# gauravchak/two_tower_models

Hardware: AMD Instinct MI355X
Metric: user-item pairs/sec (in-batch softmax train step: fwd + zero_grad + bwd + dense-exact Adam) (higher is better)
Workload: dtype f32

## Files before the change

### include/tt_hotpath.h

```cpp
#ifndef TT_HOTPATH_H
#define TT_HOTPATH_H

#include <stdint.h>

#ifdef __cplusplus
extern "C" {
#endif

#define TT_ABI_VERSION 6

#define TT_E_BADARG (-1)
#define TT_E_WORKSPACE (-2)
#define TT_E_UNSUPPORTED (-3)

typedef void* tt_stream_t;

int tt_abi_version(void);
const char* tt_last_error_string(void);

int tt_profile_enable(int on);
int tt_profile_read(const char* kernel, double* total_ms, int64_t* launches);
int tt_profile_filter(const char* kernels);
int tt_profile_pause(int paused);

int tt_gather_rows(const float* table, int64_t n_rows, int64_t dim, const int64_t* ids,
                   int64_t n_ids, float* out, int64_t ld_out, int32_t* oob_flag,
                   tt_stream_t stream);

#define TT_GEMM_NT 0
#define TT_GEMM_NN 1
#define TT_GEMM_TN 2
#define TT_EPI_NONE 0
#define TT_EPI_RELU 1
#define TT_EPI_RELU_MASK 2
int64_t tt_gemm_workspace_bytes(int layout, int64_t M, int64_t N, int64_t K);
int tt_gemm_f32(int layout, int64_t M, int64_t N, int64_t K, const float* A, int64_t lda,
                const float* B, int64_t ldb, float* C, int64_t ldc, const float* bias,
                int epilogue, const float* aux, int64_t ldaux, int accumulate, void* ws,
                int64_t ws_bytes, tt_stream_t stream);
int tt_gemm_tn_colsum_f32(int64_t M, int64_t N, int64_t K, const float* A, int64_t lda, const float* B,
                          int64_t ldb, float* C, int64_t ldc, int accumulate, float* a_colsum, void* ws,
                          int64_t ws_bytes, tt_stream_t stream);

int64_t tt_colsum_workspace_bytes(int64_t M, int64_t N);
int tt_colsum_f32(const float* X, int64_t M, int64_t N, int64_t ldx, float* out, void* ws,
                  int64_t ws_bytes, tt_stream_t stream);

typedef struct {
  const float* table; int64_t n_rows; const int64_t* ids; const float* feats; int64_t ldf; int64_t F;
  const float *W1, *b1, *W2, *b2, *W3, *b3;
  float* y; int64_t ldy; float* h_out; float* tin_out;
  const float* extra; int64_t ldx;
} tt_tower_fwd_side;
typedef struct {
  const float* dy; int64_t ldy; const float *W2, *W3, *h;
  float* d_emb; int64_t ld_demb; float* d_f; float* dh;
  float* d_extra; int64_t ld_dx;
} tt_tower_bwd_side;
typedef struct {
  const float* dy; int64_t ldy; const float *tin, *d_f, *h, *dh, *feats; int64_t ldf; int64_t F;
  float *dW1, *db1, *dW2, *db2, *dW3, *db3;
  void* ws; int64_t ws_bytes;
  const float* extra; int64_t ldx;
} tt_tower_wgrad_side;
int tt_tower_supported(int64_t D, int64_t F, int64_t hidden, int64_t d_out, int64_t E);
// ... 323 lines not shown
```

### two_tower_models_amd/_native.py

```python
from __future__ import annotations

import ctypes as C
import os
from typing import Optional

import torch

_PKG = os.path.dirname(os.path.abspath(__file__))
LIB_PATH = os.path.join(_PKG, "lib", "libtt_hotpath.so")

TT_GEMM_NT, TT_GEMM_NN, TT_GEMM_TN = 0, 1, 2
TT_EPI_NONE, TT_EPI_RELU, TT_EPI_RELU_MASK = 0, 1, 2
TT_F32, TT_BF16, TT_F16X2 = 0, 1, 2
TT_E_BADARG, TT_E_WORKSPACE, TT_E_UNSUPPORTED = -1, -2, -3
TT_DEBIAS_COMBINED, TT_DEBIAS_POSITION, TT_DEBIAS_USER = 0, 1, 2
TT_COMM_ID_BYTES = 128
TT_COMM_F32, TT_COMM_I32, TT_COMM_I64, TT_COMM_U8 = 0, 1, 2, 3
TT_COMM_SUM, TT_COMM_MAX = 0, 1
TT_MAX_GRAD_SOURCES = 4
ABI_VERSION = 6

_vp, _i64, _i32, _int = C.c_void_p, C.c_int64, C.c_int32, C.c_int


# ... 32 lines not shown
                ("extra", _vp), ("ldx", _i64)]


class TowerBwdSide(C.Structure):

    _fields_ = [("dy", _vp), ("ldy", _i64), ("W2", _vp), ("W3", _vp), ("h", _vp), ("d_emb", _vp), ("ld_demb", _i64), ("d_f", _vp),
                ("dh", _vp), ("d_extra", _vp), ("ld_dx", _i64)]


class TowerWgradSide(C.Structure):

    _fields_ = [("dy", _vp), ("ldy", _i64), ("tin", _vp), ("d_f", _vp), ("h", _vp), ("dh", _vp), ("feats", _vp), ("ldf", _i64),
                ("F", _i64), ("dW1", _vp), ("db1", _vp), ("dW2", _vp), ("db2", _vp), ("dW3", _vp), ("db3", _vp), ("ws", _vp),
                ("ws_bytes", _i64), ("extra", _vp), ("ldx", _i64)]


class PlanJob(C.Structure):

    _fields_ = [("ids", _vp), ("n_ids", _i64), ("n_rows", _i64), ("sorted_ids", _vp), ("perm", _vp), ("seg_begin", _vp), ("n_unique", _vp)]


TT_PLAN_MAX_JOBS = 4
TT_ROUTE_MAX_JOBS = 8


class RouteJob(C.Structure):

    _fields_ = [("ids", _vp), ("n_ids", _i64), ("n_rows", _i64), ("rows_per_rank", _i64), ("counts", _vp), ("max_count", _vp),
                ("ws", _vp), ("ws_bytes", _i64), ("cap", _i64), ("send_ids", _vp), ("slot_of", _vp), ("src_of", _vp)]


class RouteServeJob(C.Structure):

    _fields_ = [("ids", _vp), ("n_ids", _i64), ("lo", _i64), ("n_local", _i64), ("local", _vp), ("table", _vp), ("dtype", _int),
                ("dim", _i64), ("rows", _vp)]


SIGNATURES = {
    "tt_abi_version": (_int, []),
    "tt_last_error_string": (C.c_char_p, []),
    "tt_profile_enable": (_int, [_int]),
    "tt_profile_read": (_int, [C.c_char_p, C.POINTER(C.c_double), C.POINTER(_i64)]),
    "tt_profile_filter": (_int, [C.c_char_p]),
    "tt_profile_pause": (_int, [_int]),
    "tt_gather_rows": (_int, [_vp, _i64, _i64, _vp, _i64, _vp, _i64, _vp, _vp]),
    "tt_gemm_workspace_bytes": (_i64, [_int, _i64, _i64, _i64]),
    "tt_gemm_f32": (_int, [_int, _i64, _i64, _i64, _vp, _i64, _vp, _i64, _vp, _i64, _vp, _int, _vp,
                           _i64, _int, _vp, _i64, _vp]),
    "tt_gemm_tn_colsum_f32": (_int, [_i64, _i64, _i64, _vp, _i64, _vp, _i64, _vp, _i64, _int, _vp, _vp, _i64, _vp]),
    "tt_colsum_workspace_bytes": (_i64, [_i64, _i64]),
    "tt_colsum_f32": (_int, [_vp, _i64, _i64, _i64, _vp, _vp, _i64, _vp]),
    "tt_tower_supported": (_int, [_i64, _i64, _i64, _i64, _i64]),
    "tt_tower_fwd": (_int, [C.POINTER(TowerFwdSide), _i32, _i64, _i64, _i64, _i64, _vp, _vp]),
    "tt_tower_bwd_data": (_int, [C.POINTER(TowerBwdSide), _i32, _i64, _i64, _i64, _i64, _vp]),
    "tt_tower_bwd_weights_workspace_bytes": (_i64, [_i64, _i64, _i64, _i64, _i64]),
    "tt_tower_bwd_weights": (_int, [C.POINTER(TowerWgradSide), _i32, _i64, _i64, _i64, _i64, _vp]),
    "tt_adam_begin_ids": (_int, [_vp, _vp, _i64, C.POINTER(AdamStashJob), _i32, _vp]),
    "tt_adam_begin_ids_planes": (_int, [_vp, _vp, _i64, C.POINTER(AdamStashJob), _i32, _i32, _vp]),
    "tt_adam_tables_finish": (_int, [C.POINTER(AdamFinishJob), _i32, _vp, _vp]),
    "tt_inbatch_ce_fwd_du_loss": (_int, [_vp, _i64, _vp, _i64, _i64, _i64, _i64, _i64, _vp, _i64, _vp, _vp, _vp, _vp, _i64, _vp, _vp,
                                         _vp, _vp, _i64, _vp]),
    "tt_scale_rows_g": (_int, [_vp, _i64, _vp, _vp, _i64, _i64, _vp, _i64, _vp, _vp]),
    "tt_inbatch_ce_workspace_bytes": (_i64, [_i64, _i64, _i64]),
    "tt_inbatch_ce_fwd": (_int, [_vp, _i64, _vp, _i64, _i64, _i64, _i64, _i64, _vp, _vp, _vp, _i64, _vp]),
    "tt_inbatch_ce_bwd": (_int, [_vp, _i64, _vp, _i64, _i64, _i64, _i64, _i64, _vp, _vp, _vp, _i64, _vp,
                                 _i64, _vp, _i64, _vp]),
    "tt_inbatch_ce_fwd_du": (_int, [_vp, _i64, _vp, _i64, _i64, _i64, _i64, _i64, _vp, _vp, _vp, _i64, _vp, _i64, _vp]),
    "tt_inbatch_ce_logits_bytes": (_i64, [_i64, _i64]),
    "tt_inbatch_ce_fwd_du_keep": (_int, [_vp, _i64, _vp, _i64, _i64, _i64, _i64, _i64, _vp, _vp, _vp, _i64, _vp, _i64,
                                         _vp, _i64, _vp]),
    "tt_inbatch_ce_bwd_kept": (_int, [_vp, _i64, _i64, _i64, _i64, _i64, _vp, _vp, _vp, _i64, _vp, _i64, _vp, _i64, _vp]),
    "tt_inbatch_ce_bias_workspace_bytes": (_i64, [_i64, _i64, _i64]),
# ... 255 lines not shown
```

### two_tower_models_amd/csrc/attention_wg.hip

```cpp
#include <stdlib.h>

#include "common.hpp"

namespace tt {

typedef float f32x16 __attribute__((ext_vector_type(16)));

namespace awg {
constexpr int ROWS = 56, LD = 36, IMG = ROWS * LD;
constexpr int SLD = 68, SCR = ROWS * SLD;
constexpr int HEADS = 4, DH = 32, D = 128;
__device__ __forceinline__ int arow(int e, int h) { return (e & 3) + 8 * (e >> 2) + 4 * h; }
}

struct AttnWgArgs {
  const float* qkv;
  const float* ctx;
  const float* lse;
  const float* d_ctx;
  float* d_qkv;
  int64_t B;
  int H;
};

// ... 112 lines not shown
  float4 vf[2][4];
  auto fetch_v = [&](int64_t bb) {
    const char* __restrict__ vb = reinterpret_cast<const char*>(p.qkv + bb * H * (3 * D));
#pragma unroll
    for (int t = 0; t < 2; ++t) {
      const int j = 32 * t + r;
      const bool ok = j < H;
      const unsigned vo = (unsigned)((ok ? j : 0) * (3 * D) + 2 * D + DH * head + 4 * h2) * 4u;
#pragma unroll
      for (int g = 0; g < 4; ++g) {
        const float4 x = *reinterpret_cast<const float4*>(vb + vo + 32u * g);
        vf[t][g] = ok ? x : make_float4(0.f, 0.f, 0.f, 0.f);
      }
    }
  };
  int64_t b = blockIdx.x;
  if (b < p.B) fetch_v(b);
  __syncthreads();
  for (; b < p.B; b += gridDim.x) {
    __syncthreads();
    __syncthreads();
    const int64_t bn = b + gridDim.x;
    float* __restrict__ ob = p.d_qkv + (b * H) * (3 * D);
#pragma unroll
    for (int t = 0; t < 2; ++t) {
      const int jrow = 32 * t + r;
      const bool jvalid = jrow < H;
      const int jr = jrow < ROWS ? jrow : ROWS - 1;
      const float* const ka = Kh + jr * LD + 4 * h2;
      f32x16 dv, dk;
#pragma unroll
      for (int e = 0; e < 16; ++e) { dv[e] = 0.f; dk[e] = 0.f; }
#pragma unroll
      for (int it = 0; it < 2; ++it) {
        const int ir = (32 * it + r) < ROWS ? 32 * it + r : ROWS - 1;
        f32x16 s, dp;
#pragma unroll
        for (int e = 0; e < 16; ++e) { s[e] = 0.f; dp[e] = 0.f; }
        const float* qa = Qh + ir * LD + 4 * h2;
        const float* ga = Gh + ir * LD + 4 * h2;
#pragma unroll
        for (int g = 0; g < 4; ++g) {
          const float4 a = *reinterpret_cast<const float4*>(qa + 8 * g);
          const float4 kq = *reinterpret_cast<const float4*>(ka + 8 * g);
          const float4 c = *reinterpret_cast<const float4*>(ga + 8 * g);
          s = __builtin_amdgcn_mfma_f32_32x32x2f32(a.x, kq.x, s, 0, 0, 0);
// ... 3 lines not shown
          dp = __builtin_amdgcn_mfma_f32_32x32x2f32(c.x, vf[t][g].x, dp, 0, 0, 0);
          dp = __builtin_amdgcn_mfma_f32_32x32x2f32(c.y, vf[t][g].y, dp, 0, 0, 0);
          dp = __builtin_amdgcn_mfma_f32_32x32x2f32(c.z, vf[t][g].z, dp, 0, 0, 0);
          dp = __builtin_amdgcn_mfma_f32_32x32x2f32(c.w, vf[t][g].w, dp, 0, 0, 0);
        }
#pragma unroll
        for (int q = 0; q < 4; ++q) {
          const float4 l4 = *reinterpret_cast<const float4*>(Lh + 32 * it + 8 * q + 4 * h2);
          const float4 d4 = *reinterpret_cast<const float4*>(Dh + 32 * it + 8 * q + 4 * h2);
          const float lv[4] = {l4.x, l4.y, l4.z, l4.w}, dl[4] = {d4.x, d4.y, d4.z, d4.w};
#pragma unroll
          for (int c = 0; c < 4; ++c) {
            const int e = 4 * q + c;
            const float pe = jvalid ? __expf(s[e] - lv[c]) : 0.f;
            s[e] = pe;
            dp[e] = pe * (dp[e] - dl[c]);
          }
        }
        const float* gy = Gh + (32 * it + 4 * h2) * LD + r;
        const float* qy = Qh + (32 * it + 4 * h2) * LD + r;
#pragma unroll
        for (int e = 0; e < 16; ++e) {
          const int ro = (e & 3) + 8 * (e >> 2);
          if (it == 1 && ro + 4 >= ROWS - 32) {
            const int i = 32 + ro + 4 * h2;
            const int ic = i < ROWS ? i : ROWS - 1;
            dv = __builtin_amdgcn_mfma_f32_32x32x2f32(s[e], Gh[ic * LD + r], dv, 0, 0, 0);
            dk = __builtin_amdgcn_mfma_f32_32x32x2f32(dp[e], Qh[ic * LD + r], dk, 0, 0, 0);
          } else {
            dv = __builtin_amdgcn_mfma_f32_32x32x2f32(s[e], gy[ro * LD], dv, 0, 0, 0);
            dk = __builtin_amdgcn_mfma_f32_32x32x2f32(dp[e], qy[ro * LD], dk, 0, 0, 0);
          }
        }
        if (jrow < ROWS) {
#pragma unroll
          for (int q = 0; q < 4; ++q)
            *reinterpret_cast<float4*>(Sh + jrow * SLD + 32 * it + 8 * q + 4 * h2) =
                make_float4(dp[4 * q], dp[4 * q + 1], dp[4 * q + 2], dp[4 * q + 3]);
        }
      }
      const unsigned oc = (unsigned)((32 * t + 4 * h2) * (3 * D) + DH * head + r);
#pragma unroll
      for (int e = 0; e < 16; ++e) {
        const int ro = (e & 3) + 8 * (e >> 2);
        if (32 * t + 4 * h2 + ro < H) {
          ob[oc + (unsigned)(ro * 3 * D + 2 * D)] = dv[e];
          ob[oc + (unsigned)(ro * 3 * D + D)] = dk[e];
        }
      }
    }
    if (bn < p.B) fetch_v(bn);
    __builtin_amdgcn_wave_barrier();

#pragma unroll
    for (int it = 0; it < 2; ++it) {
      f32x16 dq;
#pragma unroll
      for (int e = 0; e < 16; ++e) dq[e] = 0.f;
      const float* sy = Sh + (4 * h2) * SLD + 32 * it + r;
      const float* ky = Kh + (4 * h2) * LD + r;
#pragma unroll
      for (int jt = 0; jt < 2; ++jt) {
#pragma unroll
        for (int e = 0; e < 16; ++e) {
          if (jt == 1 && (e >> 2) == 3) continue;
          const int ro = 32 * jt + (e & 3) + 8 * (e >> 2);
          dq = __builtin_amdgcn_mfma_f32_32x32x2f32(sy[ro * SLD], ky[ro * LD], dq, 0, 0, 0);
        }
      }
      const unsigned oc = (unsigned)((32 * it + 4 * h2) * (3 * D) + DH * head + r);
#pragma unroll
      for (int e = 0; e < 16; ++e) {
        const int ro = (e & 3) + 8 * (e >> 2);
        if (32 * it + 4 * h2 + ro < H) ob[oc + (unsigned)(ro * 3 * D)] = dq[e] * scale;
      }
    }
    __syncthreads();
  }
}

bool attn_bwd_wg_supported(const void* qkv, const void* ctx, const void* d_ctx, const void* d_qkv, int64_t H, int64_t D,
                           int64_t heads) {
  const uintptr_t al = reinterpret_cast<uintptr_t>(qkv) | reinterpret_cast<uintptr_t>(ctx) | reinterpret_cast<uintptr_t>(d_ctx) |
                       reinterpret_cast<uintptr_t>(d_qkv);
  return (al & 15) == 0 && heads == awg::HEADS && D == awg::D && H >= 1 && H <= 50;
}

int attn_bwd_wg(const float* qkv, const float* ctx, const float* lse, const float* d_ctx, int64_t B, int64_t H, float* d_qkv,
                hipStream_t st) {
  AttnWgArgs a{qkv, ctx, lse, d_ctx, d_qkv, B, (int)H};
  const unsigned grid = (unsigned)(B < 256 ? B : 256);
  ProfScope prof("attn_bwd_wg_kernel", st);
  attn_bwd_wg_kernel<<<grid, 512, 0, st>>>(a);
// ... 5 lines not shown
```

### two_tower_models_amd/csrc/gemm.hip

```cpp
#include <stdlib.h>

#include "common.hpp"

namespace tt {

typedef float f32x16 __attribute__((ext_vector_type(16)));

constexpr int BK = 32;
constexpr int LDK = BK + 4;

struct GemmArgs {
  const float* A;
  const float* B;
  float* C;
  const float* bias;
  const float* aux;
  int64_t M, N, K, lda, ldb, ldc, ldaux;
  int64_t k_per_split;
  int epilogue, accumulate, a_vec, b_vec, splits;
  float* a_colsum;
};

template <int ROWS, bool FULL>
__device__ __forceinline__ void load_kc(float4 (&st)[ROWS * 8 / 256], const float* __restrict__ X,
// ... 48 lines not shown
        const float* p = X + k * ld + row;
        if (vec && row + 3 < nrows) {
          v = *reinterpret_cast<const float4*>(p);
        } else {
          if (row + 0 < nrows) v.x = p[0];
          if (row + 1 < nrows) v.y = p[1];
          if (row + 2 < nrows) v.z = p[2];
          if (row + 3 < nrows) v.w = p[3];
        }
      }
      st[i] = v;
    }
  }
}
template <int ROWS>
__device__ __forceinline__ void store_rc(const float4 (&st)[ROWS * 8 / 256], float* Xs) {
#pragma unroll
  for (int i = 0; i < ROWS * 8 / 256; ++i) {
    const int f = threadIdx.x + 256 * i;
    *reinterpret_cast<float4*>(Xs + (f / (ROWS / 4)) * ROWS + 4 * (f % (ROWS / 4))) = st[i];
  }
}

template <int BM, int BN, bool A_KC, bool B_KC, bool FULL>
__global__ __launch_bounds__(256) void gemm_kernel(const GemmArgs g) {
  constexpr int TM = BM / 64, TN = BN / 64;
  constexpr int A_FLOATS = A_KC ? BM * LDK : BK * BM;
  constexpr int B_FLOATS = B_KC ? BN * LDK : BK * BN;
  extern __shared__ __attribute__((aligned(16))) char smem_raw[];
  float* smem = reinterpret_cast<float*>(smem_raw);
  constexpr int STAGE_FLOATS = A_FLOATS + B_FLOATS;

  const int lane = threadIdx.x & 63, wave = threadIdx.x >> 6;
  const int r = lane & 31, h = lane >> 5;
  const int wm = (wave >> 1) * (BM / 2), wn = (wave & 1) * (BN / 2);
  const int64_t m0 = (int64_t)blockIdx.y * BM, n0 = (int64_t)blockIdx.x * BN;
  const int64_t kbeg = (int64_t)blockIdx.z * g.k_per_split;
  const int64_t kend = (kbeg + g.k_per_split < g.K) ? kbeg + g.k_per_split : g.K;

  f32x16 acc[TM][TN];
#pragma unroll
  for (int i = 0; i < TM; ++i)
#pragma unroll
    for (int j = 0; j < TN; ++j)
#pragma unroll
      for (int e = 0; e < 16; ++e) acc[i][j][e] = 0.f;

  float4 sa[BM * 8 / 256], sb[BN * 8 / 256];
#define TT_FETCH(k0)                                                                              \
  do {                                                                                            \
    if constexpr (A_KC) load_kc<BM, FULL>(sa, g.A, g.lda, m0, g.M, (k0), kend, g.a_vec);          \
    else load_rc<BM, FULL>(sa, g.A, g.lda, m0, g.M, (k0), kend, g.a_vec);                         \
    if constexpr (B_KC) load_kc<BN, FULL>(sb, g.B, g.ldb, n0, g.N, (k0), kend, g.b_vec);          \
    else load_rc<BN, FULL>(sb, g.B, g.ldb, n0, g.N, (k0), kend, g.b_vec);                         \
  } while (0)
#define TT_COMMIT(buf)                                                                            \
  do {                                                                                            \
    float* a_d = smem + (buf) * STAGE_FLOATS;                                                     \
    float* b_d = a_d + A_FLOATS;                                                                  \
    if constexpr (A_KC) store_kc<BM>(sa, a_d); else store_rc<BM>(sa, a_d);                        \
    if constexpr (B_KC) store_kc<BN>(sb, b_d); else store_rc<BN>(sb, b_d);                        \
  } while (0)

  const bool do_colsum = !A_KC && g.a_colsum != nullptr && blockIdx.x == 0;
  float csum = 0.f;

  const int64_t ntiles = (kend > kbeg) ? (kend - kbeg + BK - 1) / BK : 0;
  if (ntiles > 0) {
    TT_FETCH(kbeg);
    TT_COMMIT(0);
  }
  __syncthreads();
  for (int64_t t = 0; t < ntiles; ++t) {
    const int cur = (int)(t & 1);
    if (t + 1 < ntiles) TT_FETCH(kbeg + (t + 1) * BK);
    const float* a_s = smem + cur * STAGE_FLOATS;
    const float* b_s = a_s + A_FLOATS;
    if constexpr (!A_KC) {
      if (do_colsum) {
#pragma unroll
        for (int q = 0; q < BK * BM / 256; ++q) csum += a_s[(q * (256 / BM) + threadIdx.x / BM) * BM + threadIdx.x % BM];
      }
    }
#pragma unroll
    for (int grp = 0; grp < BK / 8; ++grp) {
      float av[TM][4], bv[TN][4];
#pragma unroll
// ... 18 lines not shown
      }
#pragma unroll
      for (int c = 0; c < 4; ++c)
#pragma unroll
        for (int i = 0; i < TM; ++i)
#pragma unroll
          for (int j = 0; j < TN; ++j)
            acc[i][j] = __builtin_amdgcn_mfma_f32_32x32x2f32(av[i][c], bv[j][c], acc[i][j], 0, 0, 0);
    }
    if (t + 1 < ntiles) TT_COMMIT(cur ^ 1);
    __syncthreads();
  }
#undef TT_FETCH
#undef TT_COMMIT

  if constexpr (!A_KC) {
    if (do_colsum) {
      smem[threadIdx.x] = csum;
      __syncthreads();
      if (threadIdx.x < BM && m0 + threadIdx.x < g.M) {
        float v = 0.f;
#pragma unroll
        for (int q = 0; q < 256 / BM; ++q) v += smem[q * BM + threadIdx.x];
        g.a_colsum[(int64_t)blockIdx.z * g.M + m0 + threadIdx.x] = v;
      }
    }
  }

  const bool partial = g.splits > 1;
  float* out = partial ? g.C + (int64_t)blockIdx.z * g.M * g.N : g.C;
  const int64_t ldo = partial ? g.N : g.ldc;
#pragma unroll
  for (int i = 0; i < TM; ++i)
#pragma unroll
    for (int j = 0; j < TN; ++j) {
      const int64_t col = n0 + wn + 32 * j + r;
      if (col >= g.N) continue;
      const float bcol = (!partial && g.bias) ? g.bias[col] : 0.f;
#pragma unroll
      for (int e = 0; e < 16; ++e) {
        const int64_t row = m0 + wm + 32 * i + (e & 3) + 8 * (e >> 2) + 4 * h;
        if (row >= g.M) continue;
        float v = acc[i][j][e];
        if (!partial) {
          v += bcol;
          if (g.epilogue == TT_EPI_RELU) v = fmaxf(v, 0.f);
          else if (g.epilogue == TT_EPI_RELU_MASK) v = (g.aux[row * g.ldaux + col] > 0.f) ? v : 0.f;
          if (g.accumulate) v += out[row * ldo + col];
        }
        out[row * ldo + col] = v;
      }
    }
}

__global__ __launch_bounds__(256) void splitk_reduce_kernel(const float* __restrict__ ws, GemmArgs g, int nb_reduce,
                                                            const float* __restrict__ cs_part, float* __restrict__ cs_out) {
  if ((int)blockIdx.x >= nb_reduce) {
    __shared__ float red[4][64];
    const int c = threadIdx.x & 63, rg = threadIdx.x >> 6;
    const int64_t col = (int64_t)(blockIdx.x - nb_reduce) * 64 + c;
    float sum = 0.f;
    if (col < g.M)
      for (int64_t p = rg; p < g.splits; p += 4) sum += cs_part[p * g.M + col];
    red[rg][c] = sum;
    __syncthreads();
    if (rg == 0 && col < g.M) cs_out[col] = ((red[0][c] + red[1][c]) + red[2][c]) + red[3][c];
    return;
  }
  const int64_t total = g.M * g.N;
  for (int64_t i = (int64_t)blockIdx.x * blockDim.x + threadIdx.x; i < total;
       i += (int64_t)nb_reduce * blockDim.x) {
    const int64_t row = i / g.N, col = i % g.N;
    float v = 0.f;
    for (int s = 0; s < g.splits; ++s) v += ws[(int64_t)s * total + i];
    if (g.bias) v += g.bias[col];
// ... 63 lines not shown
template <int BM, int BN, bool A_KC, bool B_KC, bool FULL>
static int launch_gemm_v(const GemmArgs& g, hipStream_t st) {
  constexpr int A_FLOATS = A_KC ? BM * LDK : BK * BM;
  constexpr int B_FLOATS = B_KC ? BN * LDK : BK * BN;
  const size_t lds = 2 * (A_FLOATS + B_FLOATS) * sizeof(float);
  dim3 grid((unsigned)ceil_div(g.N, BN), (unsigned)ceil_div(g.M, BM), (unsigned)g.splits);
  static bool lds_opt_in = false;
  if (!lds_opt_in && lds > 64 * 1024) {
    hipError_t e = hipFuncSetAttribute(reinterpret_cast<const void*>(gemm_kernel<BM, BN, A_KC, B_KC, FULL>),
                                       hipFuncAttributeMaxDynamicSharedMemorySize, (int)lds);
    if (e != hipSuccess) { set_error("gemm_kernel: hipFuncSetAttribute: %s", hipGetErrorString(e)); return (int)e; }
    lds_opt_in = true;
  }
  gemm_kernel<BM, BN, A_KC, B_KC, FULL><<<grid, 256, lds, st>>>(g);
  return check_launch("gemm_kernel");
}
template <int BM, int BN, bool A_KC, bool B_KC>
static int launch_gemm(const GemmArgs& g, hipStream_t st) {
  const bool full = g.M % BM == 0 && g.N % BN == 0 && g.K % BK == 0 && g.a_vec && g.b_vec;
  return full ? launch_gemm_v<BM, BN, A_KC, B_KC, true>(g, st) : launch_gemm_v<BM, BN, A_KC, B_KC, false>(g, st);
}

static inline bool al16(const void* p) { return (reinterpret_cast<uintptr_t>(p) & 15) == 0; }

int gemm_ws_try(int layout, int64_t M, int64_t N, int64_t K, const float* A, int64_t lda, const float* W,
                int64_t ldw, float* C, int64_t ldc, const float* bias, int epilogue, const float* aux,
                int64_t ldaux, int accumulate, hipStream_t st);
int gemm_ws16_try(int layout, int64_t M, int64_t N, int64_t K, const float* A, int64_t lda, const float* W, int64_t ldw,
                  float* C, int64_t ldc, const float* bias, int epilogue, int accumulate, hipStream_t st);
int64_t gemm_tn_stream_ws_floats(int64_t M, int64_t N, int64_t K);
int gemm_tn_stream_try(int64_t M, int64_t N, int64_t K, const float* A, int64_t lda, const float* B, int64_t ldb,
                       float* C, int64_t ldc, int accumulate, float* a_colsum, void* ws, int64_t ws_bytes, hipStream_t st);

}

using namespace tt;

extern "C" int64_t tt_gemm_workspace_bytes(int layout, int64_t M, int64_t N, int64_t K) {
  (void)layout;
  if (M <= 0 || N <= 0 || K <= 0) return 0;
  const GemmPlan p = plan_gemm(M, N, K);
  const int64_t generic = p.splits > 1 ? round_up((int64_t)p.splits * M * (N + 1) * (int64_t)sizeof(float), 256) : 0;
  const int64_t stream = layout == TT_GEMM_TN ? round_up(gemm_tn_stream_ws_floats(M, N, K) * (int64_t)sizeof(float), 256) : 0;
  return generic > stream ? generic : stream;
}

// ... 74 lines not shown
  return gemm_impl(TT_GEMM_TN, M, N, K, A, lda, B, ldb, C, ldc, nullptr, TT_EPI_NONE, nullptr, 0, accumulate,
                   a_colsum, ws, ws_bytes, stream);
}

extern "C" int64_t tt_colsum_workspace_bytes(int64_t M, int64_t N) {
  if (M <= 0 || N <= 0) return 0;
  return round_up(ceil_div(M, colsum_rows_per_part(M)) * N * (int64_t)sizeof(float), 256);
}

extern "C" int tt_colsum_f32(const float* X, int64_t M, int64_t N, int64_t ldx, float* out, void* ws,
                             int64_t ws_bytes, tt_stream_t stream) {
  if (!X || !out) return fail_arg("tt_colsum_f32: null pointer");
  if (M <= 0 || N <= 0 || ldx < N) return fail_arg("tt_colsum_f32: sizes");
  if (!ws || ws_bytes < tt_colsum_workspace_bytes(M, N)) { set_error("tt_colsum_f32: workspace"); return TT_E_WORKSPACE; }
  const int64_t rpp = colsum_rows_per_part(M);
  const int64_t nparts = ceil_div(M, rpp);
  float* part = reinterpret_cast<float*>(ws);
  colsum_stage1<<<dim3((unsigned)ceil_div(N, 64), (unsigned)nparts), 256, 0, S(stream)>>>(X, M, N, ldx, part, rpp);
  int rc = check_launch("colsum_stage1");
  if (rc) return rc;
  colsum_stage2<<<(unsigned)ceil_div(N, 64), 256, 0, S(stream)>>>(part, nparts, N, out);
  return check_launch("colsum_stage2");
}
```

### two_tower_models_amd/ops.py

```python
from __future__ import annotations

import ctypes as C
import os
import weakref
import warnings
from typing import List, Optional, Sequence, Tuple

import torch

from . import _native as N


def _f32_2d(t: torch.Tensor, name: str) -> Tuple[int, int, int, int]:
    if t.dtype != torch.float32 or t.dim() != 2:
        raise TypeError(f"{name}: expected a 2-D float32 tensor, got {tuple(t.shape)} {t.dtype}")
    if t.size(1) > 1 and t.stride(1) != 1:
        raise ValueError(f"{name}: columns must be contiguous")
    ld = t.stride(0) if t.size(0) > 1 else max(t.size(1), t.stride(0))
    return t.data_ptr(), t.size(0), t.size(1), max(ld, t.size(1))


def _rowmajor(t: torch.Tensor) -> torch.Tensor:
    return t if (t.dim() == 2 and (t.size(1) == 1 or t.stride(1) == 1) and t.stride(0) >= t.size(1)) else t.contiguous()


def _ws(dev: torch.device, nbytes: int, slot: str = "ws") -> Tuple[Optional[int], int]:
    if nbytes <= 0:
        return None, 0
    if _aux_forks[0] and dev.type == "cuda" and torch.cuda.current_stream(dev) == N.aux_stream(dev):
        slot += "@aux"
    buf = N.scratch.get(dev, nbytes, slot)
    return buf.data_ptr(), buf.numel()


_FOLD_ASIDE = True
_EL_WGRAD_SIDE = True
_CONCURRENT_TOWERS = os.environ.get("TT_TOWERS_SERIAL") is None
_FORK_MIN_ROWS = 2048
_aux_forks = [0]


class AuxFork:

    def __init__(self, dev: torch.device, rows: int = 1 << 30):
        self.on = _CONCURRENT_TOWERS and dev.type == "cuda" and rows >= _FORK_MIN_ROWS and not torch.cuda.is_current_stream_capturing()
        if self.on:
            self.counted = torch.is_grad_enabled()
            _aux_forks[0] += 1
            self.main, self.aux = torch.cuda.current_stream(dev), N.aux_stream(dev)
            self.at = torch.cuda.Event()
            self.at.record(self.main)

    def __enter__(self):
        if self.on:
            self.aux.wait_event(self.at)
            self.ctx = torch.cuda.stream(self.aux)
            self.ctx.__enter__()
        return self

# ... 1056 lines not shown
                                       d_ue.data_ptr(), DI, N.ptr(d_pos), N.ptr(d_w), N.ptr(d_b), N.stream()),
                "tt_debias_loss_bwd")
        return d_ce, None, None, None, d_ue, d_pos, d_w, d_b, None


def fold_weights(w_in, b_in, w_po, b_po, slot: str = "ws"):
    D = w_po.shape[0]
    dev = w_in.device
    w_eff = torch.empty(3 * D, D, dtype=torch.float32, device=dev)
    gemm(N.TT_GEMM_NN, w_in, w_po, w_eff, 3 * D, D, D, slot=slot)
    b_eff = torch.empty(1, 3 * D, dtype=torch.float32, device=dev)
    gemm(N.TT_GEMM_NT, b_po.view(1, D), w_in, b_eff, 1, 3 * D, D, bias=b_in, slot=slot)
    return w_eff, b_eff.view(-1)


def fold_weight_grads(G, s, w_in, w_po, b_po, dW_in, dW_po, db_po) -> None:
    D = w_po.shape[0]
    gemm(N.TT_GEMM_NT, G, w_po, dW_in, 3 * D, D, D)
    gemm(N.TT_GEMM_NT, s.view(3 * D, 1), b_po.view(D, 1), dW_in, 3 * D, D, 1, accumulate=True)
    gemm(N.TT_GEMM_TN, w_in, G, dW_po, D, D, 3 * D)
    gemm(N.TT_GEMM_NN, s.view(1, 3 * D), w_in, db_po.view(1, D), 1, D, 3 * D)


def _attn_fwd(qkv, B, H, D, heads):
    ctx_t = torch.empty(B * H, D, dtype=torch.float32, device=qkv.device)
    lse = torch.empty(B, heads, H, dtype=torch.float32, device=qkv.device)
    N.check(N.load().tt_attn_fwd(qkv.data_ptr(), B, H, D, heads, ctx_t.data_ptr(), lse.data_ptr(), N.stream()),
            "tt_attn_fwd")
    return ctx_t, lse


class HistoryEncoder(_LookupFunction):

    @staticmethod
    def forward(ctx, source, ids, pe, heads: int, *layer_params):
        dev = N.require_device(source, ids, pe, *layer_params)
        L = len(layer_params) // 4
        lib = N.load()
        ctx.lookup_index = None
        if ids is not None:
            if ids.dtype not in (torch.int64, torch.int32):
                raise TypeError(f"user_history ids must be int64 or int32, got {ids.dtype}")
            ids = ids.to(torch.int64).contiguous()
            B, H = ids.shape
            D = source.shape[1]
            src, row_ids, ctx.lookup_index = lookup_source(source, ids, _recording(ctx))
# ... 152 lines not shown
                def last_weights(on_side, x=x, q0=q0, xbar=xbar, ctx0=ctx0, dW_in=dW_in, db_in=db_in, dW_out=dW_out, db_out=db_out,
                                 wsp=wsp, wsn=wsn):
                    N.check(lib.tt_enc_last_bwd_weights(x.data_ptr(), B, H, D, heads, d_recent.data_ptr(), 2 * D, q0.data_ptr(),
                                                        xbar.data_ptr(), ctx0.data_ptr(), dW_in.data_ptr(), db_in.data_ptr(),
                                                        dW_out.data_ptr(), db_out.data_ptr(), wsp, wsn, N.stream()),
                            "tt_enc_last_bwd_weights")

                lw = list(leaf_params[4 * l + 1: 4 * l + 4]) + ([] if l in ctx.folded else [leaf_params[4 * l]])
                w_aside = False
                if _EL_WGRAD_SIDE:
                    w_aside = run_on_side(dev, last_weights, hold=(x, q0, xbar, ctx0, d_out) + ((dW_in,) if l in ctx.folded else ()),
                                          leaves=lw)
                else:
                    last_weights(False)
                w_done = None
                if w_aside and l in ctx.folded:
                    w_done = torch.cuda.Event()
                    w_done.record(N.aux_stream(dev))
                if l in ctx.folded:
                    w_po, b_po = layer_params[4 * (l - 1) + 2], layer_params[4 * (l - 1) + 3]
                    G, dW_in = dW_in, torch.empty(3 * D, D, dtype=torch.float32, device=dev)
                    dW_po = torch.empty(D, D, dtype=torch.float32, device=dev)
                    db_po = torch.empty(D, dtype=torch.float32, device=dev)

                    def last_folded_weights(on_side, G=G, db_in=db_in, dW_in=dW_in, dW_po=dW_po, db_po=db_po, w_po=w_po, b_po=b_po,
                                            w_in=w_in):
                        fold_weight_grads(G, db_in, w_in, w_po, b_po, dW_in, dW_po, db_po)

                    tail_jobs.append((last_folded_weights, w_done))
                    prev_out_grads = (dW_po, db_po)
                grads[4 * l: 4 * l + 4] = [dW_in, db_in, dW_out, db_out]
                continue
            x, qkv, ctx_t, lse = saved[4 * l: 4 * l + 4]
            dW_out = torch.empty(D, D, dtype=torch.float32, device=dev)
            if prev_out_grads is not None:
                dW_out, db_out = prev_out_grads
                d_ctx = dx
                prev_out_grads = None
            elif l == L - 1:
                rows0 = ctx_t.view(B, H * D)[:, :D]
                _, db_out = gemm_tn_colsum(d_recent, rows0, dW_out)
                d_ctx = torch.zeros(B * H, D, dtype=torch.float32, device=dev)
                gemm(N.TT_GEMM_NN, d_recent, w_out, d_ctx.view(B, H * D)[:, :D], B, D, D)
            else:
                db_out = wgrad(dx, ctx_t, dW_out, "o", l)
                d_ctx = torch.empty(B * H, D, dtype=torch.float32, device=dev)
                gemm(N.TT_GEMM_NN, dx, w_out, d_ctx, B * H, D, D)
            d_qkv = torch.empty(B * H, 3 * D, dtype=torch.float32, device=dev)
            N.check(lib.tt_attn_bwd(qkv.data_ptr(), ctx_t.data_ptr(), lse.data_ptr(), d_ctx.data_ptr(), B, H, D,
                                    heads, d_qkv.data_ptr(), N.stream()), "tt_attn_bwd")
            dW_in = torch.empty(3 * D, D, dtype=torch.float32, device=dev)
            if l in ctx.folded:
                w_po, b_po = layer_params[4 * (l - 1) + 2], layer_params[4 * (l - 1) + 3]
                w_eff = ctx.folded[l]
                G = torch.empty(3 * D, D, dtype=torch.float32, device=dev)
                db_in = torch.empty(3 * D, dtype=torch.float32, device=dev)
                dW_po = torch.empty(D, D, dtype=torch.float32, device=dev)
                db_po = torch.empty(D, dtype=torch.float32, device=dev)

                def folded_G(on_side, d_qkv=d_qkv, x=x, G=G, db_in=db_in):
                    gemm_tn_colsum(d_qkv, x, G, db=db_in, slot="ws_side_i" if on_side else "ws")

                def folded_weights(on_side, G=G, db_in=db_in, dW_in=dW_in, dW_po=dW_po, db_po=db_po, w_po=w_po, b_po=b_po, w_in=w_in):
                    fold_weight_grads(G, db_in, w_in, w_po, b_po, dW_in, dW_po, db_po)

                hold_f = (d_qkv, x, G, w_po, b_po, w_in, w_eff)
                leaves_f = list(leaf_params[4 * l: 4 * l + 2]) + list(leaf_params[4 * (l - 1) + 2: 4 * (l - 1) + 4])
                aside = run_on_side(dev, folded_G, hold=hold_f, leaves=leaves_f)
                g_done = None
                if aside:
                    g_done = torch.cuda.Event()
                    g_done.record(N.aux_stream(dev))
                tail_jobs.append((folded_weights, g_done))
                dx = torch.empty(B * H, D, dtype=torch.float32, device=dev)
                gemm(N.TT_GEMM_NN, d_qkv, w_eff, dx, B * H, D, 3 * D)
                prev_out_grads = (dW_po, db_po)
            else:
                db_in = wgrad(d_qkv, x, dW_in, "i", l)
                dx = torch.empty(B * H, D, dtype=torch.float32, device=dev)
                rc = N.TT_E_UNSUPPORTED
                if l == 0 and not _ENC_GENERIC and w_in.is_contiguous():
                    rc = lib.tt_hist_dx_pool_bwd(d_qkv.data_ptr(), w_in.data_ptr(), B, H, D, d_pooled.data_ptr(), 2 * D, dx.data_ptr(),
                                                 N.stream())
                if rc == 0:
                    pool_done = True
                elif rc == N.TT_E_UNSUPPORTED:
                    gemm(N.TT_GEMM_NN, d_qkv, w_in, dx, B * H, D, 3 * D)
                else:
                    N.check(rc, "tt_hist_dx_pool_bwd")
            grads[4 * l: 4 * l + 4] = [dW_in, db_in, dW_out, db_out]
        for fn, g_done in tail_jobs:
            if g_done is not None:
                torch.cuda.current_stream().wait_event(g_done)
            fn(False)
        if dx is None:
            dx = torch.zeros(B * H, D, dtype=torch.float32, device=dev)
            dx.view(B, H, D)[:, 0, :].copy_(d_recent)
        if not pool_done:
            N.check(lib.tt_hist_pool_bwd(dx.data_ptr(), B, H, D, d_pooled.data_ptr(), 2 * D, N.stream()),
                    "tt_hist_pool_bwd")
        d_source = None
        if ctx.needs_input_grad[0]:
            if ctx.has_ids:
                d_source = _route_table_grad(ctx.table, ids.reshape(-1), dx, ctx.lookup_index)
            else:
                d_source = dx.view(B, H, D)
        return (d_source, None, None, None, *grads)


def mips_split_rows(x: torch.Tensor) -> Tuple[torch.Tensor, torch.Tensor]:
    dev = N.require_device(x)
    lib = N.load()
    x = x.detach().contiguous()
    if x.dtype != torch.float32 or x.dim() != 2 or x.shape[1] != 128:
        raise TypeError("split-fp16 scoring takes float32 [rows, 128]")
    out = torch.empty(x.shape[0], 2 * x.shape[1], dtype=torch.float16, device=dev)
    scale = torch.empty(1, dtype=torch.float32, device=dev)
# ... 174 lines not shown
```

Baseline: 1.516 million.

## Batch folded attention weight-grad GEMMs into one multi-job kernel launch

Adds a fold_weight_grads kernel that runs the four small GEMMs behind folded attention weight gradients (dW_in, its bias rank-1 update, dW_out, db_out) for up to four layers in a single launch. It does this by refactoring the GEMM kernel body into a reusable device tile function. The backward tail now waits on all side-stream events first and then issues one batched call, instead of several per-layer gemm launches. This cuts launch overhead for these tiny D×D matrices. Separately, the attention bwd kernel skips out-of-range MFMA steps instead of clamping indices, and hoists the per-lane output offset.

```diff
diff --git a/include/tt_hotpath.h b/include/tt_hotpath.h
--- a/include/tt_hotpath.h
+++ b/include/tt_hotpath.h
@@ -41,6 +41,14 @@
 int tt_gemm_tn_colsum_f32(int64_t M, int64_t N, int64_t K, const float* A, int64_t lda, const float* B,
                           int64_t ldb, float* C, int64_t ldc, int accumulate, float* a_colsum, void* ws,
                           int64_t ws_bytes, tt_stream_t stream);
+
+#define TT_FOLD_MAX_JOBS 4
+typedef struct {
+  const float *G, *s, *W_in, *W_o, *b_o;
+  float *dW_in, *dW_o, *db_o;
+  int64_t D;
+} tt_fold_job;
+int tt_fold_weight_grads_jobs(const tt_fold_job* jobs , int32_t n_jobs, tt_stream_t stream);
 
 int64_t tt_colsum_workspace_bytes(int64_t M, int64_t N);
 int tt_colsum_f32(const float* X, int64_t M, int64_t N, int64_t ldx, float* out, void* ws,
diff --git a/two_tower_models_amd/_native.py b/two_tower_models_amd/_native.py
--- a/two_tower_models_amd/_native.py
+++ b/two_tower_models_amd/_native.py
@@ -78,6 +78,13 @@
 
 TT_PLAN_MAX_JOBS = 4
 TT_ROUTE_MAX_JOBS = 8
+TT_FOLD_MAX_JOBS = 4
+
+
+class FoldJob(C.Structure):
+
+    _fields_ = [("G", _vp), ("s", _vp), ("W_in", _vp), ("W_o", _vp), ("b_o", _vp), ("dW_in", _vp), ("dW_o", _vp), ("db_o", _vp),
+                ("D", _i64)]
 
 
 class RouteJob(C.Structure):
@@ -104,6 +111,7 @@
     "tt_gemm_f32": (_int, [_int, _i64, _i64, _i64, _vp, _i64, _vp, _i64, _vp, _i64, _vp, _int, _vp,
                            _i64, _int, _vp, _i64, _vp]),
     "tt_gemm_tn_colsum_f32": (_int, [_i64, _i64, _i64, _vp, _i64, _vp, _i64, _vp, _i64, _int, _vp, _vp, _i64, _vp]),
+    "tt_fold_weight_grads_jobs": (_int, [C.POINTER(FoldJob), _i32, _vp]),
     "tt_colsum_workspace_bytes": (_i64, [_i64, _i64]),
     "tt_colsum_f32": (_int, [_vp, _i64, _i64, _i64, _vp, _vp, _i64, _vp]),
     "tt_tower_supported": (_int, [_i64, _i64, _i64, _i64, _i64]),
diff --git a/two_tower_models_amd/csrc/attention_wg.hip b/two_tower_models_amd/csrc/attention_wg.hip
--- a/two_tower_models_amd/csrc/attention_wg.hip
+++ b/two_tower_models_amd/csrc/attention_wg.hip
@@ -158,6 +158,8 @@
     __syncthreads();
     const int64_t bn = b + gridDim.x;
     float* __restrict__ ob = p.d_qkv + (b * H) * (3 * D);
+    unsigned lane_oc = (unsigned)(4 * h2 * (3 * D) + DH * head + r);
+    asm volatile("" : "+v"(lane_oc));
 #pragma unroll
     for (int t = 0; t < 2; ++t) {
       const int jrow = 32 * t + r;
@@ -207,15 +209,9 @@
 #pragma unroll
         for (int e = 0; e < 16; ++e) {
           const int ro = (e & 3) + 8 * (e >> 2);
-          if (it == 1 && ro + 4 >= ROWS - 32) {
-            const int i = 32 + ro + 4 * h2;
-            const int ic = i < ROWS ? i : ROWS - 1;
-            dv = __builtin_amdgcn_mfma_f32_32x32x2f32(s[e], Gh[ic * LD + r], dv, 0, 0, 0);
-            dk = __builtin_amdgcn_mfma_f32_32x32x2f32(dp[e], Qh[ic * LD + r], dk, 0, 0, 0);
-          } else {
-            dv = __builtin_amdgcn_mfma_f32_32x32x2f32(s[e], gy[ro * LD], dv, 0, 0, 0);
-            dk = __builtin_amdgcn_mfma_f32_32x32x2f32(dp[e], qy[ro * LD], dk, 0, 0, 0);
-          }
+          if (it == 1 && ro + 32 >= ROWS) continue;
+          dv = __builtin_amdgcn_mfma_f32_32x32x2f32(s[e], gy[ro * LD], dv, 0, 0, 0);
+          dk = __builtin_amdgcn_mfma_f32_32x32x2f32(dp[e], qy[ro * LD], dk, 0, 0, 0);
         }
         if (jrow < ROWS) {
 #pragma unroll
@@ -224,7 +220,7 @@
                 make_float4(dp[4 * q], dp[4 * q + 1], dp[4 * q + 2], dp[4 * q + 3]);
         }
       }
-      const unsigned oc = (unsigned)((32 * t + 4 * h2) * (3 * D) + DH * head + r);
+      const unsigned oc = lane_oc + (unsigned)(32 * t * (3 * D));
 #pragma unroll
       for (int e = 0; e < 16; ++e) {
         const int ro = (e & 3) + 8 * (e >> 2);
@@ -253,7 +249,7 @@
           dq = __builtin_amdgcn_mfma_f32_32x32x2f32(sy[ro * SLD], ky[ro * LD], dq, 0, 0, 0);
         }
       }
-      const unsigned oc = (unsigned)((32 * it + 4 * h2) * (3 * D) + DH * head + r);
+      const unsigned oc = lane_oc + (unsigned)(32 * it * (3 * D));
 #pragma unroll
       for (int e = 0; e < 16; ++e) {
         const int ro = (e & 3) + 8 * (e >> 2);
diff --git a/two_tower_models_amd/csrc/gemm.hip b/two_tower_models_amd/csrc/gemm.hip
--- a/two_tower_models_amd/csrc/gemm.hip
+++ b/two_tower_models_amd/csrc/gemm.hip
@@ -94,20 +94,18 @@
   }
 }
 
-template <int BM, int BN, bool A_KC, bool B_KC, bool FULL>
-__global__ __launch_bounds__(256) void gemm_kernel(const GemmArgs g) {
+template <int BM, int BN, bool A_KC, bool B_KC, bool FULL_A, bool FULL_B>
+__device__ __forceinline__ void gemm_tile(const GemmArgs g, const unsigned bx, const unsigned by, const unsigned bz, float* smem) {
   constexpr int TM = BM / 64, TN = BN / 64;
   constexpr int A_FLOATS = A_KC ? BM * LDK : BK * BM;
   constexpr int B_FLOATS = B_KC ? BN * LDK : BK * BN;
-  extern __shared__ __attribute__((aligned(16))) char smem_raw[];
-  float* smem = reinterpret_cast<float*>(smem_raw);
   constexpr int STAGE_FLOATS = A_FLOATS + B_FLOATS;
 
   const int lane = threadIdx.x & 63, wave = threadIdx.x >> 6;
   const int r = lane & 31, h = lane >> 5;
   const int wm = (wave >> 1) * (BM / 2), wn = (wave & 1) * (BN / 2);
-  const int64_t m0 = (int64_t)blockIdx.y * BM, n0 = (int64_t)blockIdx.x * BN;
-  const int64_t kbeg = (int64_t)blockIdx.z * g.k_per_split;
+  const int64_t m0 = (int64_t)by * BM, n0 = (int64_t)bx * BN;
+  const int64_t kbeg = (int64_t)bz * g.k_per_split;
   const int64_t kend = (kbeg + g.k_per_split < g.K) ? kbeg + g.k_per_split : g.K;
 
   f32x16 acc[TM][TN];
@@ -121,10 +119,10 @@
   float4 sa[BM * 8 / 256], sb[BN * 8 / 256];
 #define TT_FETCH(k0)                                                                              \
   do {                                                                                            \
-    if constexpr (A_KC) load_kc<BM, FULL>(sa, g.A, g.lda, m0, g.M, (k0), kend, g.a_vec);          \
-    else load_rc<BM, FULL>(sa, g.A, g.lda, m0, g.M, (k0), kend, g.a_vec);                         \
-    if constexpr (B_KC) load_kc<BN, FULL>(sb, g.B, g.ldb, n0, g.N, (k0), kend, g.b_vec);          \
-    else load_rc<BN, FULL>(sb, g.B, g.ldb, n0, g.N, (k0), kend, g.b_vec);                         \
+    if constexpr (A_KC) load_kc<BM, FULL_A>(sa, g.A, g.lda, m0, g.M, (k0), kend, g.a_vec);        \
+    else load_rc<BM, FULL_A>(sa, g.A, g.lda, m0, g.M, (k0), kend, g.a_vec);                       \
+    if constexpr (B_KC) load_kc<BN, FULL_B>(sb, g.B, g.ldb, n0, g.N, (k0), kend, g.b_vec);        \
+    else load_rc<BN, FULL_B>(sb, g.B, g.ldb, n0, g.N, (k0), kend, g.b_vec);                       \
   } while (0)
 #define TT_COMMIT(buf)                                                                            \
   do {                                                                                            \
@@ -134,7 +132,7 @@
     if constexpr (B_KC) store_kc<BN>(sb, b_d); else store_rc<BN>(sb, b_d);                        \
   } while (0)
 
-  const bool do_colsum = !A_KC && g.a_colsum != nullptr && blockIdx.x == 0;
+  const bool do_colsum = !A_KC && g.a_colsum != nullptr && bx == 0;
   float csum = 0.f;
 
   const int64_t ntiles = (kend > kbeg) ? (kend - kbeg + BK - 1) / BK : 0;
@@ -199,13 +197,13 @@
         float v = 0.f;
 #pragma unroll
         for (int q = 0; q < 256 / BM; ++q) v += smem[q * BM + threadIdx.x];
-        g.a_colsum[(int64_t)blockIdx.z * g.M + m0 + threadIdx.x] = v;
+        g.a_colsum[(int64_t)bz * g.M + m0 + threadIdx.x] = v;
       }
     }
   }
 
   const bool partial = g.splits > 1;
-  float* out = partial ? g.C + (int64_t)blockIdx.z * g.M * g.N : g.C;
+  float* out = partial ? g.C + (int64_t)bz * g.M * g.N : g.C;
   const int64_t ldo = partial ? g.N : g.ldc;
 #pragma unroll
   for (int i = 0; i < TM; ++i)
@@ -228,6 +226,12 @@
         out[row * ldo + col] = v;
       }
     }
+}
+
+template <int BM, int BN, bool A_KC, bool B_KC, bool FULL>
+__global__ __launch_bounds__(256) void gemm_kernel(const GemmArgs g) {
+  extern __shared__ __attribute__((aligned(16))) char smem_raw[];
+  gemm_tile<BM, BN, A_KC, B_KC, FULL, FULL>(g, blockIdx.x, blockIdx.y, blockIdx.z, reinterpret_cast<float*>(smem_raw));
 }
 
 __global__ __launch_bounds__(256) void splitk_reduce_kernel(const float* __restrict__ ws, GemmArgs g, int nb_reduce,
@@ -337,6 +341,57 @@
 }
 
 static inline bool al16(const void* p) { return (reinterpret_cast<uintptr_t>(p) & 15) == 0; }
+
+constexpr int FOLD_MAX_JOBS = TT_FOLD_MAX_JOBS;
+struct FoldJobs {
+  const float* G[FOLD_MAX_JOBS];
+  const float* s[FOLD_MAX_JOBS];
+  const float* W_in[FOLD_MAX_JOBS];
+  const float* W_o[FOLD_MAX_JOBS];
+  const float* b_o[FOLD_MAX_JOBS];
+  float* dW_in[FOLD_MAX_JOBS];
+  float* dW_o[FOLD_MAX_JOBS];
+  float* db_o[FOLD_MAX_JOBS];
+  int D;
+};
+constexpr int FOLD_LDS_BYTES = 2 * (64 * LDK + 64 * LDK) * (int)sizeof(float);
+
+template <bool FULL>
+__global__ __launch_bounds__(256) void fold_weight_grads_kernel(const FoldJobs jobs) {
+  extern __shared__ __attribute__((aligned(16))) char smem_raw[];
+  float* smem = reinterpret_cast<float*>(smem_raw);
+  const int D = jobs.D;
+  const unsigned td = (unsigned)(D + 63) / 64, t3 = (unsigned)(3 * D + 63) / 64;
+  const unsigned n_in = t3 * td, n_o = td * td, per_job = n_in + n_o + td;
+  const unsigned q = blockIdx.x / per_job;
+  unsigned t = blockIdx.x % per_job;
+  GemmArgs g;
+  g.bias = nullptr; g.aux = nullptr; g.ldaux = 0; g.epilogue = TT_EPI_NONE; g.accumulate = 0;
+  g.a_vec = 1; g.b_vec = 1; g.splits = 1; g.a_colsum = nullptr;
+  if (t < n_in) {
+    g.A = jobs.G[q]; g.B = jobs.W_o[q]; g.C = jobs.dW_in[q];
+    g.M = 3 * D; g.N = D; g.K = D; g.lda = D; g.ldb = D; g.ldc = D;
+    g.k_per_split = (D + BK - 1) / BK * BK;
+    gemm_tile<64, 64, true, true, FULL, FULL>(g, t % td, t / td, 0, smem);
+    g.A = jobs.s[q]; g.B = jobs.b_o[q];
+    g.K = 1; g.lda = 1; g.ldb = 1; g.k_per_split = BK; g.a_vec = 0; g.b_vec = 0; g.accumulate = 1;
+    gemm_tile<64, 64, true, true, false, false>(g, t % td, t / td, 0, smem);
+    return;
+  }
+  t -= n_in;
+  g.k_per_split = (3 * D + BK - 1) / BK * BK;
+  g.K = 3 * D; g.N = D; g.ldb = D; g.ldc = D;
+  if (t < n_o) {
+    g.A = jobs.W_in[q]; g.B = jobs.G[q]; g.C = jobs.dW_o[q];
+    g.M = D; g.lda = D;
+    gemm_tile<64, 64, false, false, FULL, FULL>(g, t % td, t / td, 0, smem);
+    return;
+  }
+  t -= n_o;
+  g.A = jobs.s[q]; g.B = jobs.W_in[q]; g.C = jobs.db_o[q];
+  g.M = 1; g.lda = 3 * D;
+  gemm_tile<64, 64, true, false, false, FULL>(g, t, 0, 0, smem);
+}
 
 int gemm_ws_try(int layout, int64_t M, int64_t N, int64_t K, const float* A, int64_t lda, const float* W,
                 int64_t ldw, float* C, int64_t ldc, const float* bias, int epilogue, const float* aux,
@@ -457,3 +512,32 @@
   colsum_stage2<<<(unsigned)ceil_div(N, 64), 256, 0, S(stream)>>>(part, nparts, N, out);
   return check_launch("colsum_stage2");
 }
+
+extern "C" int tt_fold_weight_grads_jobs(const tt_fold_job* jobs, int32_t n_jobs, tt_stream_t stream) {
+  if (!jobs || n_jobs <= 0 || n_jobs > TT_FOLD_MAX_JOBS) return fail_arg("tt_fold_weight_grads_jobs: jobs");
+  FoldJobs a{};
+  uintptr_t al = 0;
+  for (int i = 0; i < n_jobs; ++i) {
+    const tt_fold_job& j = jobs[i];
+    if (!j.G || !j.s || !j.W_in || !j.W_o || !j.b_o || !j.dW_in || !j.dW_o || !j.db_o)
+      return fail_arg("tt_fold_weight_grads_jobs: null pointer");
+    if (j.D <= 0) return fail_arg("tt_fold_weight_grads_jobs: sizes");
+    al |= reinterpret_cast<uintptr_t>(j.G) | reinterpret_cast<uintptr_t>(j.s) | reinterpret_cast<uintptr_t>(j.W_in) |
+          reinterpret_cast<uintptr_t>(j.W_o) | reinterpret_cast<uintptr_t>(j.b_o) | reinterpret_cast<uintptr_t>(j.dW_in) |
+          reinterpret_cast<uintptr_t>(j.dW_o) | reinterpret_cast<uintptr_t>(j.db_o);
+    a.G[i] = j.G; a.s[i] = j.s; a.W_in[i] = j.W_in; a.W_o[i] = j.W_o; a.b_o[i] = j.b_o;
+    a.dW_in[i] = j.dW_in; a.dW_o[i] = j.dW_o; a.db_o[i] = j.db_o;
+  }
+  const int64_t D = jobs[0].D;
+  for (int i = 1; i < n_jobs; ++i)
+    if (jobs[i].D != D) { set_error("tt_fold_weight_grads_jobs: one D per call"); return TT_E_UNSUPPORTED; }
+  if (D != 32 && D != 64 && D != 128) { set_error("tt_fold_weight_grads_jobs: D = %lld not in {32, 64, 128}", (long long)D); return TT_E_UNSUPPORTED; }
+  if (al & 15) { set_error("tt_fold_weight_grads_jobs: operands must be 16-byte aligned"); return TT_E_UNSUPPORTED; }
+  a.D = (int)D;
+  const unsigned td = (unsigned)ceil_div(D, 64), t3 = (unsigned)ceil_div(3 * D, 64);
+  const unsigned blocks = (unsigned)n_jobs * (t3 * td + td * td + td);
+  hipStream_t st = S(stream);
+  if (D % 64 == 0) fold_weight_grads_kernel<true><<<blocks, 256, FOLD_LDS_BYTES, st>>>(a);
+  else fold_weight_grads_kernel<false><<<blocks, 256, FOLD_LDS_BYTES, st>>>(a);
+  return check_launch("fold_weight_grads_kernel");
+}
diff --git a/two_tower_models_amd/ops.py b/two_tower_models_amd/ops.py
--- a/two_tower_models_amd/ops.py
+++ b/two_tower_models_amd/ops.py
@@ -35,6 +35,7 @@
 
 _FOLD_ASIDE = True
 _EL_WGRAD_SIDE = True
+_FOLD_GRADS_ONE_LAUNCH = True
 _CONCURRENT_TOWERS = os.environ.get("TT_TOWERS_SERIAL") is None
 _FORK_MIN_ROWS = 2048
 _aux_forks = [0]
@@ -1137,6 +1138,27 @@
     gemm(N.TT_GEMM_NN, s.view(1, 3 * D), w_in, db_po.view(1, D), 1, D, 3 * D)
 
 
+def fold_weight_grads_jobs(jobs) -> None:
+    if not jobs:
+        return
+    D = jobs[0][3].shape[0]
+    one = (_FOLD_GRADS_ONE_LAUNCH and D in (32, 64, 128)
+           and all(t.is_contiguous() and t.data_ptr() % 16 == 0 and t.dtype == torch.float32 for j in jobs for t in j)
+           and all(j[3].shape[0] == D for j in jobs))
+    if not one:
+        for j in jobs:
+            fold_weight_grads(*j)
+        return
+    lib = N.load()
+    for i in range(0, len(jobs), N.TT_FOLD_MAX_JOBS):
+        part = jobs[i: i + N.TT_FOLD_MAX_JOBS]
+        arr = (N.FoldJob * len(part))()
+        for a, j in zip(arr, part):
+            a.G, a.s, a.W_in, a.W_o, a.b_o, a.dW_in, a.dW_o, a.db_o = (t.data_ptr() for t in j)
+            a.D = D
+        N.check(lib.tt_fold_weight_grads_jobs(arr, len(part), N.stream()), "tt_fold_weight_grads_jobs")
+
+
 def _attn_fwd(qkv, B, H, D, heads):
     ctx_t = torch.empty(B * H, D, dtype=torch.float32, device=qkv.device)
     lse = torch.empty(B, heads, H, dtype=torch.float32, device=qkv.device)
@@ -1335,12 +1357,7 @@
                     G, dW_in = dW_in, torch.empty(3 * D, D, dtype=torch.float32, device=dev)
                     dW_po = torch.empty(D, D, dtype=torch.float32, device=dev)
                     db_po = torch.empty(D, dtype=torch.float32, device=dev)
-
-                    def last_folded_weights(on_side, G=G, db_in=db_in, dW_in=dW_in, dW_po=dW_po, db_po=db_po, w_po=w_po, b_po=b_po,
-                                            w_in=w_in):
-                        fold_weight_grads(G, db_in, w_in, w_po, b_po, dW_in, dW_po, db_po)
-
-                    tail_jobs.append((last_folded_weights, w_done))
+                    tail_jobs.append(((G, db_in, w_in, w_po, b_po, dW_in, dW_po, db_po), w_done))
                     prev_out_grads = (dW_po, db_po)
                 grads[4 * l: 4 * l + 4] = [dW_in, db_in, dW_out, db_out]
                 continue
@@ -1374,9 +1391,6 @@
                 def folded_G(on_side, d_qkv=d_qkv, x=x, G=G, db_in=db_in):
                     gemm_tn_colsum(d_qkv, x, G, db=db_in, slot="ws_side_i" if on_side else "ws")
 
-                def folded_weights(on_side, G=G, db_in=db_in, dW_in=dW_in, dW_po=dW_po, db_po=db_po, w_po=w_po, b_po=b_po, w_in=w_in):
-                    fold_weight_grads(G, db_in, w_in, w_po, b_po, dW_in, dW_po, db_po)
-
                 hold_f = (d_qkv, x, G, w_po, b_po, w_in, w_eff)
                 leaves_f = list(leaf_params[4 * l: 4 * l + 2]) + list(leaf_params[4 * (l - 1) + 2: 4 * (l - 1) + 4])
                 aside = run_on_side(dev, folded_G, hold=hold_f, leaves=leaves_f)
@@ -1384,7 +1398,7 @@
                 if aside:
                     g_done = torch.cuda.Event()
                     g_done.record(N.aux_stream(dev))
-                tail_jobs.append((folded_weights, g_done))
+                tail_jobs.append(((G, db_in, w_in, w_po, b_po, dW_in, dW_po, db_po), g_done))
                 dx = torch.empty(B * H, D, dtype=torch.float32, device=dev)
                 gemm(N.TT_GEMM_NN, d_qkv, w_eff, dx, B * H, D, 3 * D)
                 prev_out_grads = (dW_po, db_po)
@@ -1402,10 +1416,10 @@
                 else:
                     N.check(rc, "tt_hist_dx_pool_bwd")
             grads[4 * l: 4 * l + 4] = [dW_in, db_in, dW_out, db_out]
-        for fn, g_done in tail_jobs:
+        for _, g_done in tail_jobs:
             if g_done is not None:
                 torch.cuda.current_stream().wait_event(g_done)
-            fn(False)
+        fold_weight_grads_jobs([operands for operands, _ in tail_jobs])
         if dx is None:
             dx = torch.zeros(B * H, D, dtype=torch.float32, device=dev)
             dx.view(B, H, D)[:, 0, :].copy_(d_recent)
```

Result: no change. 1.516 million (median of 3 runs) (-0.0%).
